# Victarry/Image-Generation-models

Measured on AMD Instinct MI355X. Metric: ddpm_cifar10_32x32_train_images_per_sec, higher is better.
Workload: dtype bf16; 1 GPU; DDPM CIFAR-10 32x32, UNet 128/1-2-4, T=1000 (BASELINE configs[1]): train step B=128/GPU + hipGraph denoise step B=64; per_gpu_batch=128, global_batch=128, parallelism=dp1, step_launch=hipGraph replay, denoise_batch=64, rccl_ranks=1, state_finite=True, matmul=bf16 MFMA, fp32 accumulate

## Files before the change

image-generation-models_amd/csrc/conv3x3_halo.hip:

```cpp
#include <stdlib.h>
#include "common.h"

#ifdef MI_HALO_TIMING
__device__ unsigned long long g_halo_ts[5 * 4096];
#define MI_TS(k) do { if (threadIdx.x == 0 && blockIdx.y == 0 && blockIdx.z == 0 && blockIdx.x < 4096) g_halo_ts[(k) * 4096 + blockIdx.x] = wall_clock64(); } while (0)
extern "C" int mi_debug_halo_ts(unsigned long long* host_out) {
    return (int)hipMemcpyFromSymbol(host_out, HIP_SYMBOL(g_halo_ts), sizeof(g_halo_ts));
}
#else
#define MI_TS(k) do {} while (0)
#endif
#ifdef MI_HALO_TAPTIME
__device__ unsigned long long g_halo_tap[4096 * 8 * 5];
extern "C" int mi_debug_halo_tap(unsigned long long* host_out) {
    return (int)hipMemcpyFromSymbol(host_out, HIP_SYMBOL(g_halo_tap), sizeof(g_halo_tap));
}
#define MI_TAP_BARRIER() do { const unsigned long long b0_ = __builtin_amdgcn_s_memtime(); __syncthreads(); \
        const unsigned long long b1_ = __builtin_amdgcn_s_memtime(); tt_work += b0_ - tt_prev; tt_bar += b1_ - b0_; tt_prev = b1_; ++tt_n; } while (0)
#else
#define MI_TAP_BARRIER() __syncthreads()
#endif
#ifndef MI_HALO_STORE_FIRST
#define MI_HALO_STORE_FIRST 1
#endif
// ... 617 lines not shown
    if (skew_env && KS == 3 && (a.W == 8 || a.W == 16)) {
        const int rows = a.TI * (a.TH + 2);
        if (a.HP * PITCH + rows * HaloSkew<CK>::EL <= MAXHP * PITCH) a.skew = HaloSkew<CK>::EL;
    }
    dim3 grid((a.N * a.H * a.W + BM - 1) / BM, (a.Nc + 127) / 128, a.ksplit);
    a.qmap = 0; a.gx = (int)grid.x; a.gy = (int)grid.y;
    static const int q_env = (int)mi_knob("MI_HALO_PQ", 1);
    if (q_env && KS == 3 && !SK && a.ksplit == 1 && !a.xmap && a.gy > 1 && a.TH == a.H) {
        const int Q = (a.gy % 2 == 0) ? 2 : 1, P = 8 / Q;
        if (Q > 1 && a.gx % P == 0) { a.qmap = Q; grid = dim3(grid.x * grid.y, 1, 1); }
    }
    if (q_env && KS == 1 && !SK && a.ksplit == 1 && a.gy > 1 && a.gx % 8 == 0) { a.qmap = 1; grid = dim3(grid.x * grid.y, 1, 1); }
    static MiPerDevice once;
    once.run([] {
        (void)hipFuncSetAttribute((const void*)conv3x3_halo_kernel<BM, CK, KS, SK, IO, WAVES, FUSE, PIPE, N64>, hipFuncAttributeMaxDynamicSharedMemorySize, 160 * 1024); });
    hipLaunchKernelGGL((conv3x3_halo_kernel<BM, CK, KS, SK, IO, WAVES, FUSE, PIPE, N64>), grid, dim3(HaloCfg<BM, WAVES>::NT), lds, st, a);
}

struct PackEntry { long long off; int taps, ci, co, tile0, frag, pad_; };

constexpr int PACK_TILE = 64;

__global__ __launch_bounds__(256) void pack_weights_kernel(const PackEntry* __restrict__ ents, int nent,
                                                           const float* __restrict__ master, uint16_t* __restrict__ wd,
                                                           uint16_t* __restrict__ wf, uint16_t* __restrict__ wdq,
                                                           uint16_t* __restrict__ wfq) {
    __shared__ float tile[PACK_TILE][PACK_TILE + 1];
    int e = 0;
    for (int hi = nent; hi - e > 1;) {
        const int mid = (e + hi) >> 1;
        if ((int)blockIdx.x >= ents[mid].tile0) e = mid; else hi = mid;
    }
    const PackEntry en = ents[e];
    int local = blockIdx.x - en.tile0;
    const int tci = (en.ci + PACK_TILE - 1) / PACK_TILE, tco = (en.co + PACK_TILE - 1) / PACK_TILE;
    int tap = local / (tci * tco);
    int rem = local - tap * (tci * tco);
    int bi = rem / tco, bj = rem - bi * tco;
    const float* src = master + en.off + (size_t)tap * en.ci * en.co;
    uint16_t* d1 = wd + en.off + (size_t)tap * en.ci * en.co;
    uint16_t* d2 = wf + en.off + (size_t)tap * en.ci * en.co;
    if (((en.ci | en.co) & 3) == 0 && (en.off & 3) == 0) {
        const int c4 = (threadIdx.x & 15) * 4, r0 = threadIdx.x >> 4;
#pragma unroll
        for (int p = 0; p < 4; ++p) {
            const int r = r0 + 16 * p, i = bi * PACK_TILE + r, j = bj * PACK_TILE + c4;
            f32x4 v = {0.f, 0.f, 0.f, 0.f};
            if (i < en.ci && j < en.co) {
                v = *reinterpret_cast<const f32x4*>(src + (size_t)i * en.co + j);
                *reinterpret_cast<u32x2*>(d1 + (size_t)i * en.co + j) = u32x2{pack_bf16(v.x, v.y), pack_bf16(v.z, v.w)};
            }
            tile[r][c4] = v.x; tile[r][c4 + 1] = v.y; tile[r][c4 + 2] = v.z; tile[r][c4 + 3] = v.w;
        }
        __syncthreads();
#pragma unroll
        for (int p = 0; p < 4; ++p) {
            const int r = r0 + 16 * p, j = bj * PACK_TILE + r, i = bi * PACK_TILE + c4;
            if (i < en.ci && j < en.co)
                *reinterpret_cast<u32x2*>(d2 + (size_t)j * en.ci + i) =
                    u32x2{pack_bf16(tile[c4][r], tile[c4 + 1][r]), pack_bf16(tile[c4 + 2][r], tile[c4 + 3][r])};
        }
        if (en.frag && wdq) {
            const int l = threadIdx.x & 63;
            const size_t tapo = (size_t)en.off + (size_t)tap * en.ci * en.co;
#pragma unroll
            for (int h = 0; h < 2; ++h) {
                const int f = (threadIdx.x >> 6) + 4 * h;
                const int r32 = (f >> 2) * 32 + (l & 31), c8 = (f & 3) * 16 + 8 * (l >> 5);
                {
                    const size_t fo = ((size_t)(bi * 2 + (f >> 2)) * (en.co / 16) + bj * 4 + (f & 3)) * 512 + l * 8;
                    *reinterpret_cast<u32x4*>(wdq + tapo + fo) =
                        u32x4{pack_bf16(tile[r32][c8], tile[r32][c8 + 1]), pack_bf16(tile[r32][c8 + 2], tile[r32][c8 + 3]),
                              pack_bf16(tile[r32][c8 + 4], tile[r32][c8 + 5]), pack_bf16(tile[r32][c8 + 6], tile[r32][c8 + 7])};
                }
                {
                    const size_t fo = ((size_t)(bj * 2 + (f >> 2)) * (en.ci / 16) + bi * 4 + (f & 3)) * 512 + l * 8;
                    *reinterpret_cast<u32x4*>(wfq + tapo + fo) =
                        u32x4{pack_bf16(tile[c8][r32], tile[c8 + 1][r32]), pack_bf16(tile[c8 + 2][r32], tile[c8 + 3][r32]),
                              pack_bf16(tile[c8 + 4][r32], tile[c8 + 5][r32]), pack_bf16(tile[c8 + 6][r32], tile[c8 + 7][r32])};
                }
            }
        }
        return;
    }
    const int tx = threadIdx.x & 63, ty = threadIdx.x >> 6;
    for (int r = ty; r < PACK_TILE; r += 4) {
        int i = bi * PACK_TILE + r, j = bj * PACK_TILE + tx;
        float v = (i < en.ci && j < en.co) ? src[(size_t)i * en.co + j] : 0.f;
        tile[r][tx] = v;
        if (i < en.ci && j < en.co) d1[(size_t)i * en.co + j] = (uint16_t)(pack_bf16(v, 0.f) & 0xffff);
    }
    __syncthreads();
    for (int r = ty; r < PACK_TILE; r += 4) {
        int j = bj * PACK_TILE + r, i = bi * PACK_TILE + tx;
        if (i < en.ci && j < en.co) d2[(size_t)j * en.ci + i] = (uint16_t)(pack_bf16(tile[tx][r], 0.f) & 0xffff);
    }
}

}

static bool halo_geom(const MiConvDesc* d, int BM, int* TH, int* TI) {
    int W = d->OW, H = d->OH;
    if (BM % W) return false;
    int rows = BM / W;
    if (rows <= H) { if (H % rows) return false; *TH = rows; *TI = 1; }
    else { if (rows % H) return false; *TH = H; *TI = rows / H; if ((long)d->N % *TI) return false; }
    int maxhp = BM == 256 ? 400 : (BM == 128 ? 288 : 160);
    return *TI * (*TH + 2) * (W + 2) <= maxhp;
}

static bool halo_ok(const MiConvDesc* d, int* bm, int* ck) {
    const bool k3 = d->KH == 3 && d->KW == 3 && d->pad == 1, k1 = d->KH == 1 && d->KW == 1 && d->pad == 0;
    if (!(k3 || k1) || d->stride != 1 || d->mode != 1) return false;
    if (d->IH != d->OH || d->IW != d->OW) return false;
    if (d->K % 32 || d->K1 % 32 || d->Nc % 4) return false;
    if (k1) {
        const long M = (long)d->N * d->OH * d->OW, nt = (d->Nc + 127) / 128;
// ... 256 lines not shown
    hipStream_t st = (hipStream_t)stream;
#define MI_FUSE_GO(IOV) \
    do { if (BM == 256 && CK == 64) launch_halo<256, 64, 3, false, IOV, 8, true>(a, st); \
         else if (BM == 256) launch_halo<256, 32, 3, false, IOV, 8, true>(a, st); \
         else if (BM == 128) launch_halo<128, 32, 3, false, IOV, 4, true>(a, st); \
         else if (CK == 64) launch_halo<64, 64, 3, false, IOV, 4, true>(a, st); \
         else launch_halo<64, 32, 3, false, IOV, 4, true>(a, st); } while (0)
    if (io == 0) MI_FUSE_GO(0); else MI_FUSE_GO(3);
#undef MI_FUSE_GO
    MI_LAUNCH_CHECK();
    return 0;
}

extern "C" int mi_conv3x3_bf16w_tile(const MiConvDesc* d, int io, int* bm, int* ck, int* sk) {
    MI_REQUIRE(d && bm && ck && sk, "null argument");
    MI_REQUIRE(halo_ok(d, bm, ck), "descriptor not supported by the halo kernel");
    int th, ti;
    *sk = (!(io & 2) && halo_splitk(d, *bm, &th, &ti)) ? 1 : 0;
    if (*sk) { *bm = 256; *ck = 64; }
    else if (halo_w8(d, *bm, &th, &ti)) { *bm = 128; *ck = 64; }
    else if (halo_wide64(d, *bm)) *ck = 64;
    return 0;
}

extern "C" int mi_conv3x3_bf16w_supported(const MiConvDesc* d) {
    int bm, ck;
    return (d && halo_ok(d, &bm, &ck)) ? 1 : 0;
}

extern "C" int mi_pack_weights_tile(void) { return PACK_TILE; }

extern "C" int mi_pack_weights_bf16(int nent, const void* entries_dev, int total_tiles, const float* master,
                                    void* wd_bf16, void* wf_bf16, void* wdq_bf16, void* wfq_bf16, void* stream) {
    MI_REQUIRE(nent > 0 && entries_dev && total_tiles > 0 && master && wd_bf16 && wf_bf16, "bad argument");
    MI_REQUIRE((wdq_bf16 == nullptr) == (wfq_bf16 == nullptr), "fragment-order copies: both or neither");
    MI_REQUIRE((((uintptr_t)wdq_bf16 | (uintptr_t)wfq_bf16) & 15) == 0, "fragment-order copies must be 16-byte aligned");
    hipLaunchKernelGGL(pack_weights_kernel, dim3(total_tiles), dim3(256), 0, (hipStream_t)stream,
                       (const PackEntry*)entries_dev, nent, master, (uint16_t*)wd_bf16, (uint16_t*)wf_bf16,
                       (uint16_t*)wdq_bf16, (uint16_t*)wfq_bf16);
    MI_LAUNCH_CHECK();
    return 0;
}
```

image-generation-models_amd/src/models/ddpm.py:

```python
from __future__ import annotations

import math
import os
from functools import partial
from typing import Dict, List, Optional, Sequence, Tuple

import numpy as np
import torch
from torch import nn

from ..ops import functional as K
from .base import BaseModel, ValidationResult

_HEADS, _DHEAD = 4, 32
_GN_GROUPS = 8


def _mode_id(name: str) -> int:
    if name not in ("fp32", "bf16"):
        raise ValueError(f"compute mode must be 'fp32' or 'bf16', got {name!r}")
    return K.MODE_BF16 if name == "bf16" else K.MODE_FP32


class _Entry:
# ... 194 lines not shown
        self.compute_mode = os.environ.get("MI_DDPM_MODE", "fp32")
        self.block_storage = os.environ.get("MI_DDPM_STORAGE", "bf16")
        self.fuse_gn_conv = os.environ.get("MI_DDPM_FUSE_GN", "auto")
        self.s2_wgrad_tr = K.debug_knob("MI_DDPM_S2_TR", "1") != "0"
        self.final_block16 = K.debug_knob("MI_DDPM_FINAL16", "1") != "0"
        self.ends16 = K.debug_knob("MI_DDPM_ENDS16", "1") != "0"
        self.dual_out = K.debug_knob("MI_DDPM_DUAL_OUT", "1") != "0"
        self.fuse_ln_qkv = K.debug_knob("MI_DDPM_FUSE_LN", "1") != "0"
        self.fuse_ln_qkv_train = K.debug_knob("MI_DDPM_FUSE_LN_TRAIN", "1") != "0"
        self.small_cin_dual = K.debug_knob("MI_DDPM_CIN_DUAL", "1") != "0"
        self.cin_dual_chores = K.debug_knob("MI_DDPM_CIN_CHORES", "1") != "0"
        self.fold_attn = K.debug_knob("MI_DDPM_FOLD_ATTN", "0") == "1"
        self.small_cout_bwd1 = K.debug_knob("MI_DDPM_COUT_BWD1", "1") != "0"
        self.fuse_final = K.debug_knob("MI_DDPM_FUSE_FINAL", "1") != "0"
        self.grad_store = K.debug_knob("MI_DDPM_GRAD_STORE", "1") != "0"
        self.accumulate_grads = False
        self.grad_ready_hook = None

        flat = torch.zeros(arch.flat_numel)
        for e in arch.entries:
            if e.init == "kaiming":
                w = torch.empty(e.shape)
                nn.init.kaiming_uniform_(w, a=math.sqrt(5))
                e.logical_view(flat).copy_(w)
            elif e.init == "ubias":
                bound = 1 / math.sqrt(e.fan_in) if e.fan_in > 0 else 0
                e.logical_view(flat).copy_(torch.empty(e.shape).uniform_(-bound, bound))
            elif e.init == "one":
                e.logical_view(flat).fill_(1.0)
        object.__setattr__(self, "_flat", flat)
        object.__setattr__(self, "_gflat", None)
        object.__setattr__(self, "_dirty", 0)
        object.__setattr__(self, "_shadow", None)
        object.__setattr__(self, "_shadow_key", None)
        object.__setattr__(self, "_shadow32", None)
        object.__setattr__(self, "_shadow32_key", None)
        object.__setattr__(self, "_zero_tab", None)
        object.__setattr__(self, "_zero_tab_retired", [])
        object.__setattr__(self, "_anchor", torch.zeros(1, requires_grad=True))
        self._plist: List[Tuple[_Entry, nn.Parameter]] = []
        for e in sorted(arch.entries, key=lambda q: q.rank):
            parts = e.key.split(".")
            node = self
            for name in parts[:-1]:
                if name not in node._modules:
                    node.add_module(name, _Node())
                node = node._modules[name]
            p = nn.Parameter(e.logical_view(flat))
            node.register_parameter(parts[-1], p)
            self._plist.append((e, p))
        self._bind(flat)

    def _bind(self, flat: torch.Tensor):
        object.__setattr__(self, "_flat", flat)
        sv = {}
        for e, p in self._plist:
            p.data = e.logical_view(flat)
            sv[e.key] = e.storage_view(flat)
        object.__setattr__(self, "_sv", sv)
        object.__setattr__(self, "_offs", {e.key: e.offset for e, _ in self._plist})
        object.__setattr__(self, "_shadow_key", None)
        object.__setattr__(self, "_shadow32_key", None)
        g = self._gflat
        if g is not None and (g.device != flat.device or g.dtype != flat.dtype):
            object.__setattr__(self, "_gflat", None)
            for _, p in self._plist:
                p.grad = None

    def _apply(self, fn, recurse=True):
        new = fn(self._flat)
        if new.dtype != torch.float32:
            raise RuntimeError("the MI355X UNet keeps fp32 master weights; use compute_mode='bf16' for bf16 math")
        if new is not self._flat:
            self._bind(new)
        return self

    @property
    def flat_params(self) -> torch.Tensor:
        return self._flat

    def mark_params_dirty(self):
        object.__setattr__(self, "_dirty", self._dirty + 1)

    def _shadows(self):
        flat = self._flat
        key = (flat.data_ptr(), flat._version, self._dirty)
        if self._shadow_key != key:
            if self._shadow is None or self._shadow[0].device != flat.device:
                ents = []
                for e in self._arch.entries:
                    if e.layout in ("conv", "convT"):
                        kh, kw, ci, co = e.storage_view(flat).shape
                        ents.append((e.offset, kh * kw, ci, co))
                table, nent, tiles = K.pack_table(ents, flat.device)
                bufs = [torch.zeros(flat.numel(), device=flat.device, dtype=torch.bfloat16) for _ in range(4)]
                object.__setattr__(self, "_shadow", (*bufs, table, nent, tiles))
            wd, wf, wdq, wfq, table, nent, tiles = self._shadow
            K.pack_weights_bf16(table, nent, tiles, flat, wd, wf, wdq, wfq)
            object.__setattr__(self, "_shadow_key", key)
        return self._shadow[:4]

    def _shadows32(self):
        flat = self._flat
        key = (flat.data_ptr(), flat._version, self._dirty)
        if getattr(self, "_shadow32_key", None) != key:
            if getattr(self, "_shadow32", None) is None or self._shadow32[0].device != flat.device:
                ents = []
                for e in self._arch.entries:
                    if e.layout in ("conv", "convT"):
                        kh, kw, ci, co = e.storage_view(flat).shape
                        ents.append((e.offset, kh * kw, ci, co))
                table, nent, tiles = K.pack_table(ents, flat.device)
                bufs = [torch.zeros(flat.numel(), device=flat.device, dtype=torch.float32) for _ in range(2)]
                object.__setattr__(self, "_shadow32", (*bufs, table, nent, tiles))
            wdq32, wfq32, table, nent, tiles = self._shadow32
            K.pack_weights_f32frag(table, nent, tiles, flat, wdq32, wfq32)
            object.__setattr__(self, "_shadow32_key", key)
        return self._shadow32[:2]

    @property
    def flat_grads(self) -> torch.Tensor:
        if self._gflat is None:
            g = torch.zeros_like(self._flat)
            object.__setattr__(self, "_gflat", g)
            gv = {}
            for e, p in self._plist:
                p.grad = e.logical_view(g)
                gv[e.key] = e.storage_view(g)
            object.__setattr__(self, "_gv", gv)
            self._build_zero_table(g.device)
        return self._gflat

    def _build_zero_table(self, device):
        skip = []
        for e in self._arch.entries:
            if e.layout in ("conv", "convT"):
                kh, kw, ci, co = e.storage_view(self._flat).shape
                if ci % 64 == 0 and co >= 32:
                    skip.append((e.offset, e.numel, e.key))
        skip.sort()
        ranges, pos = [], 0
        for off, numel, _ in skip:
            if off > pos:
                ranges.append((pos, off - pos))
            pos = off + numel
        if self._arch.flat_numel > pos:
            ranges.append((pos, self._arch.flat_numel - pos))
        if self._zero_tab is not None:
            self._zero_tab_retired.append(self._zero_tab)
        table = torch.tensor(ranges, dtype=torch.int64).reshape(-1, 2).to(device)
        object.__setattr__(self, "_zero_tab", (table, len(ranges), frozenset(k for _, _, k in skip)))

    def zero_grad(self, set_to_none: bool = False):
        if self._gflat is not None:
            self._gflat.zero_()

    def load_state_dict(self, state_dict, strict: bool = True, assign: bool = False):
        out = super().load_state_dict(state_dict, strict=strict, assign=False)
        return out

    def forward(self, x, time):
        if not x.is_cuda:
            raise RuntimeError("Unet.forward: input is not on a HIP device; this implementation has no CPU path")
        if self._flat.device != x.device:
            raise RuntimeError("Unet parameters and input are on different devices; call .to(device) first")
        if torch.is_grad_enabled() and (self.training or x.requires_grad):
            if self._anchor.device != x.device:
                object.__setattr__(self, "_anchor", torch.zeros(1, device=x.device, requires_grad=True))
            return _UnetFunction.apply(x, time, self._anchor, self)
        y, _ = self._execute(x, time, record=False)
        return y

    def _execute(self, x, time, record):
        x_in = K.nchw_to_nhwc(x.float())
        eps, tape = self.forward_nhwc(x_in, time, record)
        return K.nhwc_to_nchw(eps), tape

    @torch.no_grad()
    def time_bias_table(self, timesteps: int) -> torch.Tensor:
        A, sv, flat = self._arch, self._sv, self._flat
        if not A.with_time:
            return None
        T = int(timesteps)
        t = torch.arange(T, device=flat.device, dtype=torch.long)

        def lin(inp, w, b):
            o, i = w.shape
            y = K.small_gemm(False, True, inp, w, bias=b)
            if y is not None:
                return y
            return K.conv_igemm(inp.view(T, 1, 1, i), w, kh=1, kw=1, stride=1, pad=0, transposed=False, w_kn=False,
# ... 818 lines not shown
```

image-generation-models_amd/src/ops/functional.py:

```python
from __future__ import annotations

import ctypes as C
import functools
import os
from typing import Optional, Tuple

import torch

from .lib import ROWSUM_MAX, WGRAD_STORE, MiConvDesc, MiGnDesc, MiRowSum, MiWgradDesc, check, load_library

MODE_FP32, MODE_BF16 = 0, 1


def debug_knob(name: str, default: str) -> str:
    if os.environ.get("MI_DEBUG_KNOBS") == "1":
        return os.environ.get(name, default)
    return default
PROBE = None


CONV_AUTO = os.environ.get("MI_CONV_AUTO", "1") == "1"


USE_CONV_PW = CONV_AUTO and debug_knob("MI_CONV_PW", "1") == "1"
# ... 54 lines not shown
def _probe_open():
    if PROBE is None:
        return None
    e0 = torch.cuda.Event(enable_timing=True)
    e0.record()
    return e0


def _probe_close(e0, sym, flops, desc, nbytes=0.0):
    e1 = torch.cuda.Event(enable_timing=True)
    e1.record()
    PROBE.append((sym, float(flops), e0, e1, desc, float(nbytes)))


def _esz(t) -> int:
    return 0 if t is None else t.element_size()


def _stream() -> C.c_void_p:
    global LAUNCHES
    LAUNCHES += 1
    return C.c_void_p(_raw_stream(_cur_dev()))


LAUNCHES = 0


_cur_dev = torch._C._cuda_getDevice
_raw_stream = torch._C._cuda_getCurrentRawStream


def _p(t: Optional[torch.Tensor]) -> C.c_void_p:
    return C.c_void_p(0 if t is None else t.data_ptr())


def _need_gpu(t: torch.Tensor):
    if not t.is_cuda:
        raise RuntimeError("libmi_ddpm kernels need tensors on an MI355X (HIP) device; there is no CPU fallback")
    if t.dtype not in (torch.float32, torch.bfloat16):
        raise RuntimeError(f"expected float32 (or bf16 block-internal storage), got {t.dtype}")
    if t.device.index != _cur_dev():
        raise RuntimeError(f"tensor is on {t.device} but the current HIP device is cuda:{torch.cuda.current_device()}; "
                           "call torch.cuda.set_device(tensor.device) first (one process per GPU)")
    if t.device.index not in _SPLITK_WS:
        _splitk_workspace(t.device)


_SPLITK_WS = {}
SPLITK_MB = int(debug_knob("MI_CONV_PW_SPLITK_MB", "64"))


def _splitk_workspace(device):
    ws = None
    if SPLITK_MB > 0 and USE_CONV_PW and not torch.cuda.is_current_stream_capturing():
        ws = torch.zeros(SPLITK_MB << 20, dtype=torch.uint8, device=device)
        torch.cuda.current_stream().synchronize()
        check(load_library().mi_conv_pw_set_splitk_workspace(ws.data_ptr(), ws.numel()), "mi_conv_pw_set_splitk_workspace")
    elif torch.cuda.is_current_stream_capturing():
        return
    _SPLITK_WS[device.index] = ws


def ld_of(t: torch.Tensor) -> int:
    if t.dim() == 2:
        assert t.stride(1) == 1
        return t.stride(0)
# ... 50 lines not shown
    if e0 is not None:
        pxt, ncls = C.c_int(), C.c_int()
        load_library().mi_conv_gt_tile(C.byref(d), C.byref(pxt), C.byref(ncls))
        flops = 2.0 * N * OH * OW * Nc * K * (kh * kw if not (transposed and stride > 1) else kh * kw / (stride * stride))
        nb = N * IH * IW * K * _esz(x) + N * OH * OW * Nc * _esz(out) * (2 if accumulate else 1) + kh * kw * K * Nc * _esz(x)
        _probe_close(e0, f"conv_gt_kernel<{'true' if _b16(out) else 'false'}, {pxt.value}{', true' if mode == MODE_FP32 else ''}>", flops,
                     f"N{N} {IH}x{IW}->{OH}x{OW} K{K}->{Nc} k{kh} s{stride} T{int(transposed)} acc{int(accumulate)}", nb)
    return (out, y16) if want16 else out


def conv_igemm(x, w, *, kh, kw, stride, pad, transposed, w_kn, K, Nc, out_hw, mode, x2=None,
               bias=None, residual=None, out=None, accumulate=False, wb=None):
    _need_gpu(x)
    N, IH, IW, K1 = x.shape
    if x2 is None:
        K1 = K
    OH, OW = out_hw
    if out is None:
        assert not accumulate
        out = new_act(N, OH, OW, Nc if Nc % 4 == 0 else (Nc + 3) // 4 * 4, x)
        if out.shape[3] != Nc:
            out.zero_()
            out = out[..., :Nc]
    d = MiConvDesc(N=N, IH=IH, IW=IW, OH=OH, OW=OW, K=K, Nc=Nc, KH=kh, KW=kw, stride=stride, pad=pad,
                   transposed=int(transposed), w_kn=int(w_kn), mode=mode, K1=K1, ldx=ld_of(x),
                   ldx2=ld_of(x2) if x2 is not None else 0, ldy=ld_of(out),
                   ldr=ld_of(residual) if residual is not None else 0, accumulate=int(accumulate))
    if PROBE is not None:
        bm, bn = C.c_int(), C.c_int()
        load_library().mi_conv_igemm_tile(C.byref(d), C.byref(bm), C.byref(bn))
        flops = 2.0 * N * OH * OW * Nc * K * (kh * kw if not (transposed and stride > 1) else kh * kw / (stride * stride))
        e0 = _probe_open()
    in16 = _b16(x)
    if in16:
        if wb is None or mode != MODE_BF16 or (x2 is not None and not _b16(x2)) or not load_library().mi_conv_igemm_bf16w_io_supported(C.byref(d)):
            raise RuntimeError("bf16-stored activations: layer not supported (check igemm_bf16_in_supported first)")
        check(load_library().mi_conv_igemm_bf16w_io(C.byref(d), _p(x), _p(x2), _p(wb), _p(bias), _p(residual), _p(out), 1, _stream()),
              "mi_conv_igemm_bf16w_io")
    elif wb is not None and mode == MODE_BF16 and K % 8 == 0:
        check(load_library().mi_conv_igemm_bf16w(C.byref(d), _p(x), _p(x2), _p(wb), _p(bias), _p(residual), _p(out), _stream()),
              "mi_conv_igemm_bf16w")
    else:
        check(load_library().mi_conv_igemm(C.byref(d), _p(x), _p(x2), _p(w), _p(bias), _p(residual), _p(out), _stream()),
              "mi_conv_igemm")
    if PROBE is not None:
        fast = wb is not None and mode == MODE_BF16 and K % 8 == 0
        nb = N * IH * IW * K * _esz(x) + N * OH * OW * Nc * _esz(out) * (2 if accumulate else 1) + kh * kw * K * Nc * (2 if fast else 4)
        _probe_close(e0, f"igemm{'_fast' if fast else ''}_kernel<{mode},{bm.value},{bn.value}{',in16' if in16 else ''}>", flops,
                     f"N{N} {IH}x{IW}->{OH}x{OW} K{K}->{Nc} k{kh} s{stride} T{int(transposed)} acc{int(accumulate)}", nb)
    return out


def conv3x3_bf16w(x, wsh, *, K, Nc, flip, ksize=3, x2=None, bias=None, residual=None, out=None, accumulate=False,
                  out_dtype=torch.float32, gn_sums=None, want16=False, wq=None):
    _need_gpu(x)
    N, H, W, K1 = x.shape
    if x2 is None:
        K1 = K
    d = MiConvDesc(N=N, IH=H, IW=W, OH=H, OW=W, K=K, Nc=Nc, KH=ksize, KW=ksize, stride=1, pad=ksize // 2, transposed=int(flip),
                   w_kn=0, mode=MODE_BF16, K1=K1, ldx=ld_of(x), ldx2=ld_of(x2) if x2 is not None else 0, ldy=0,
                   ldr=ld_of(residual) if residual is not None else 0, accumulate=int(accumulate))
    lib = load_library()
    if not _query("mi_conv3x3_bf16w_supported", d):
        return None
    if out is None:
        assert not accumulate
# ... 33 lines not shown
        pt = _query("mi_conv3x3_pw_x32_tile", d)
        if pt and (N * H * W // pt) * ((Nc + 127) // 128) >= PW_MIN_TILES:
            assert gn_sums is None or (gn_sums.dtype == torch.int64 and gn_sums.numel() == N * (Nc // 16) * 2)
            e0 = _probe_open()
            check(lib.mi_conv3x3_pw_x32(C.byref(d), _p(x), _p(x2), _p(wq), _p(bias), _p(residual), _p(out), _b16(out), _p(gn_sums), _stream()),
                  "mi_conv3x3_pw_x32")
            if e0 is not None:
                nb = (N * H * W * K * 4 + N * H * W * Nc * (_esz(out) * (2 if accumulate else 1) + _esz(residual)) + 9 * K * Nc * 2)
                _probe_close(e0, f"conv_pw_kernel<{'true' if _b16(out) else 'false'}, {0 if gn_sums is None else 1}, 0, {_pw_tile_now(d, 0, True, pt)}, true>",
                             2.0 * N * H * W * Nc * K * 9, f"N{N} {H}x{W} K{K}{'(2src)' if x2 is not None else ''}->{Nc} fp32 in flip{int(flip)} acc{int(accumulate)}", nb)
            return out
    if (gn_sums is not None and ksize == 3 and _b16(x) and USE_CONV_PW and wq is not None and _pick_pw(N, H, W, K, Nc, d)
            and _query("mi_conv3x3_pw_supported", d)):
        assert gn_sums.dtype == torch.int64 and gn_sums.numel() == N * (Nc // 16) * 2
        e0 = _probe_open()
        check(lib.mi_conv3x3_pw_gnsums(C.byref(d), _p(x), _p(x2), _p(wq), _p(bias), _p(residual), _p(out), _b16(out), _p(gn_sums), _stream()),
              "mi_conv3x3_pw_gnsums")
        if e0 is not None:
            nb = (N * H * W * K * 2 + N * H * W * Nc * (_esz(out) * (2 if accumulate else 1) + _esz(residual)) + 9 * K * Nc * 2)
            _probe_close(e0, _pw_sym(d, _b16(out), 1), 2.0 * N * H * W * Nc * K * 9,
                         f"N{N} {H}x{W} K{K}->{Nc} + GroupNorm sums", nb)
        return out
    if gn_sums is None and not want16 and ksize == 3 and _b16(x):
        if USE_CONV_PW and wq is not None and _pick_pw(N, H, W, K, Nc, d):
            pick = "pw"
    if pick == "pw":
        e0 = _probe_open()
        check(lib.mi_conv3x3_pw(C.byref(d), _p(x), _p(x2), _p(wq), _p(bias), _p(residual), _p(out), _b16(out), _stream()), "mi_conv3x3_pw")
        if e0 is not None:
            nb = (N * H * W * K * 2 + N * H * W * Nc * (_esz(out) * (2 if accumulate else 1) + _esz(residual)) + 9 * K * Nc * 2)
            _probe_close(e0, _pw_sym(d, _b16(out)), 2.0 * N * H * W * Nc * K * 9,
                         f"N{N} {H}x{W} K{K}{'(2src)' if x2 is not None else ''}->{Nc} flip{int(flip)} acc{int(accumulate)}", nb)
        return out
    e0 = _probe_open()
    if want16:
        assert out.dtype == torch.float32 and gn_sums is None and not accumulate
        y16 = new_act(N, H, W, Nc, x, torch.bfloat16)
        check(lib.mi_conv3x3_bf16w_io_dual(C.byref(d), _p(x), _p(x2), _p(wsh), _p(bias), _p(residual), _p(out), _p(y16), ld_of(y16), io, _stream()),
              "mi_conv3x3_bf16w_io_dual")
    elif gn_sums is not None:
        assert ksize == 3 and gn_sums.dtype == torch.int64 and gn_sums.numel() == N * (Nc // 16) * 2
        check(lib.mi_conv3x3_bf16w_io_gnsums(C.byref(d), _p(x), _p(x2), _p(wsh), _p(bias), _p(residual), _p(out), io, _p(gn_sums), _stream()),
              "mi_conv3x3_bf16w_io_gnsums")
    elif io:
        check(lib.mi_conv3x3_bf16w_io(C.byref(d), _p(x), _p(x2), _p(wsh), _p(bias), _p(residual), _p(out), io, _stream()),
              "mi_conv3x3_bf16w_io")
    else:
        check(lib.mi_conv3x3_bf16w(C.byref(d), _p(x), _p(x2), _p(wsh), _p(bias), _p(residual), _p(out), _stream()),
              "mi_conv3x3_bf16w")
    if e0 is not None:
        bm, ck, sk = C.c_int(), C.c_int(), C.c_int()
        lib.mi_conv3x3_bf16w_tile(C.byref(d), io, C.byref(bm), C.byref(ck), C.byref(sk))
        nb = (N * H * W * K * _esz(x) + N * H * W * Nc * (_esz(out) * (2 if accumulate else 1) + _esz(residual))
              + ksize * ksize * K * Nc * 2)
        _probe_close(e0, f"conv3x3_halo_kernel<{bm.value}, {ck.value}, {ksize}, {'true' if sk.value else 'false'}, {io}, {8 if bm.value == 256 or (bm.value == 128 and ck.value == 64) else 4}>",
                     2.0 * N * H * W * Nc * K * ksize * ksize,
                     f"N{N} {H}x{W} K{K}{'(2src)' if x2 is not None else ''}->{Nc} flip{int(flip)} acc{int(accumulate)} io{io}", nb)
    return (out, y16) if want16 else out


def gn_stats_coef(x, gamma, beta, *, groups=8, eps=1e-5, temb=None):
    _need_gpu(x)
    N, H, W, Cc = x.shape
    stats = torch.empty((N, groups, 2), device=x.device, dtype=torch.float32)
    coef = torch.empty((3, N, Cc), device=x.device, dtype=torch.float32)
    d = MiGnDesc(N=N, HW=H * W, C=Cc, G=groups, eps=eps, ldx=ld_of(x), ldy=Cc, ldr=0)
# ... 95 lines not shown
                                                 _stream()), "mi_conv3x3_pw_gn_mish_sums")
        else:
            check(lib.mi_conv3x3_pw_gn_mish(C.byref(d), _p(x), _p(coef), _p(wq), _p(bias), _p(y), _b16(y), _stream()), "mi_conv3x3_pw_gn_mish")
        if e0 is not None:
            _probe_close(e0, f"conv_pw_kernel<{'true' if _b16(y) else 'false'}, {3 if coef is None else 2}, 0, {_pw_tile_now(d, 2, False, ptf)}>", 2.0 * N * H * W * Nc * K * 9,
                         f"N{N} {H}x{W} K{K}->{Nc} fused GN+Mish", N * H * W * (K * 2 + Nc * _esz(y)) + 9 * K * Nc * 2)
        return y
    if ptf and x.dtype == torch.float32:
        y = new_act(N, H, W, Nc, x, x.dtype if out_dtype is None else out_dtype)
        d.ldy = Nc
        e0 = _probe_open()
        if coef is None and (K // gn[4]) not in (16, 32, 64):
            _, coef = gn_coef_from_sums(gn[0], N, H * W, gn[1], gn[2], groups=gn[4], eps=gn[5], temb=gn[3])
        if coef is None:
            sums, gamma, beta, temb, groups, eps = gn
            check(lib.mi_conv3x3_pw_x32_gn_mish_sums(C.byref(d), _p(x), _p(sums), _p(gamma), _p(beta), _p(temb),
                                                     ld_of(temb) if temb is not None else 0, groups, eps, _p(wq), _p(bias), _p(y), _b16(y),
                                                     _stream()), "mi_conv3x3_pw_x32_gn_mish_sums")
        else:
            check(lib.mi_conv3x3_pw_x32_gn_mish(C.byref(d), _p(x), _p(coef), _p(wq), _p(bias), _p(y), _b16(y), _stream()),
                  "mi_conv3x3_pw_x32_gn_mish")
        if e0 is not None:
            _probe_close(e0, f"conv_pw_kernel<{'true' if _b16(y) else 'false'}, {3 if coef is None else 2}, 0, {_pw_tile_now(d, 2, True, ptf)}, true>",
                         2.0 * N * H * W * Nc * K * 9, f"N{N} {H}x{W} K{K}->{Nc} fused GN+Mish, fp32 in",
                         N * H * W * (K * 4 + Nc * _esz(y)) + 9 * K * Nc * 2)
        return y
    if not lib.mi_conv3x3_gn_mish_supported(C.byref(d)):
        return None
    out_dtype = x.dtype if out_dtype is None else out_dtype
    if out_dtype != x.dtype:
        raise RuntimeError("the fused kernel writes y in x's storage type (fp32 -> fp32 or bf16 -> bf16)")
    y = new_act(N, H, W, Nc, x, out_dtype)
    io = 3 if x.dtype == torch.bfloat16 else 0
    e0 = _probe_open()
    if gn is not None:
        sums, gamma, beta, temb, groups, eps = gn
        check(lib.mi_conv3x3_gn_mish_sums(C.byref(d), _p(x), _p(sums), _p(gamma), _p(beta), _p(temb), ld_of(temb) if temb is not None else 0,
                                          groups, eps, _p(wsh), _p(bias), _p(y), io, _stream()), "mi_conv3x3_gn_mish_sums")
    else:
        check(lib.mi_conv3x3_gn_mish(C.byref(d), _p(x), _p(coef), _p(wsh), _p(bias), _p(y), io, _stream()), "mi_conv3x3_gn_mish")
    if e0 is not None:
        bm, ck = C.c_int(), C.c_int()
        lib.mi_conv3x3_gn_mish_tile(C.byref(d), C.byref(bm), C.byref(ck))
        _probe_close(e0, f"conv3x3_halo_kernel<{bm.value}, {ck.value}, 3, false, {io}, {8 if bm.value == 256 else 4}, true>",
                     2.0 * N * H * W * Nc * K * 9, f"N{N} {H}x{W} K{K}->{Nc} fused GN+Mish",
                     N * H * W * (K * _esz(x) + Nc * _esz(y)) + 9 * K * Nc * 2)
    return y


def pack_weights_tile():
    return int(load_library().mi_pack_weights_tile())


PACK_ENTRY = [("off", "<i8"), ("taps", "<i4"), ("ci", "<i4"), ("co", "<i4"), ("tile0", "<i4"), ("frag", "<i4"), ("pad", "<i4")]


def pack_table(entries, device):
    import numpy as np
    rec = np.zeros(len(entries), dtype=np.dtype(PACK_ENTRY))
    tile, T = 0, pack_weights_tile()
    for i, (off, taps, ci, co) in enumerate(entries):
        rec[i] = (off, taps, ci, co, tile, int(taps in (1, 9, 16) and ci % 64 == 0 and co % 64 == 0), 0)
        tile += taps * ((ci + T - 1) // T) * ((co + T - 1) // T)
    return torch.from_numpy(rec.view(np.uint8).copy()).to(device), len(entries), tile


def pack_weights_bf16(table_dev, nent, total_tiles, master, wd, wf, wdq=None, wfq=None):
    e0 = _probe_open()
    check(load_library().mi_pack_weights_bf16(nent, _p(table_dev), total_tiles, _p(master), _p(wd), _p(wf), _p(wdq), _p(wfq), _stream()),
          "mi_pack_weights_bf16")
    if e0 is not None:
        _probe_close(e0, "pack_weights_kernel", 0.0, f"{master.numel()} params", master.numel() * (8.0 if wdq is None else 12.0))


def pack_weights_f32frag(table_dev, nent, total_tiles, master, wdq32, wfq32):
    e0 = _probe_open()
    check(load_library().mi_pack_weights_f32frag(nent, _p(table_dev), total_tiles, _p(master), _p(wdq32), _p(wfq32), _stream()),
          "mi_pack_weights_f32frag")
    if e0 is not None:
        _probe_close(e0, "pack_f32frag_kernel", 0.0, f"{master.numel()} params", master.numel() * 12.0)


def conv3x3_f32(x, wq32, *, K, Nc, flip, x2=None, bias=None, residual=None, out=None, accumulate=False):
    _need_gpu(x)
    if x.dtype != torch.float32 or (x2 is not None and x2.dtype != torch.float32) or not USE_CONV_PW:
        return None
    N, H, W, K1 = x.shape
    if x2 is None:
        K1 = K
    d = MiConvDesc(N=N, IH=H, IW=W, OH=H, OW=W, K=K, Nc=Nc, KH=3, KW=3, stride=1, pad=1, transposed=int(flip),
                   w_kn=0, mode=MODE_FP32, K1=K1, ldx=ld_of(x), ldx2=ld_of(x2) if x2 is not None else 0, ldy=Nc,
                   ldr=ld_of(residual) if residual is not None else 0, accumulate=int(accumulate))
    pt = _query("mi_conv3x3_pw_f32_tile", d)
    if not pt:
        return None
    if out is None:
        assert not accumulate
        out = new_act(N, H, W, Nc, x, torch.float32)
    d.ldy = ld_of(out)
    if d.ldy % 8:
        return None
    e0 = _probe_open()
    check(load_library().mi_conv3x3_pw_f32(C.byref(d), _p(x), _p(x2), _p(wq32), _p(bias), _p(residual), _p(out), _stream()), "mi_conv3x3_pw_f32")
    if e0 is not None:
        nb = (N * H * W * K * 4 + N * H * W * Nc * (4 * (2 if accumulate else 1) + _esz(residual)) + 9 * K * Nc * 4)
# ... 674 lines not shown
    M, D = src_rows.shape
    check(load_library().mi_vq_scatter_rows(M, D, table.shape[0], _p(src_rows), src_rows.stride(0), _p(idx), _p(table), _stream()),
          "mi_vq_scatter_rows")


def linattn_fwd(qkv, heads=4):
    _need_gpu(qkv)
    N, H, W, C3 = qkv.shape
    assert C3 == 3 * heads * 32 and qkv.is_contiguous()
    out = new_act(N, H, W, heads * 32, qkv, qkv.dtype)
    ctx = torch.empty((N, heads, 32, 32), device=qkv.device, dtype=torch.float32)
    kstat = torch.empty((N, heads, 32, 2), device=qkv.device, dtype=torch.float32)
    e0 = _probe_open()
    lib = load_library()
    need = _linattn_ws(N, H * W, heads)
    ws = _workspace(qkv.device, need) if need else None
    check(lib.mi_linattn_fwd_ws(N, H * W, heads, _p(qkv), _p(out), _p(ctx), _p(kstat), _b16(qkv), _p(ws), ws.numel() * 4 if need else 0,
                                _stream()), "mi_linattn_fwd")
    if e0 is not None:
        _probe_close(e0, f"linattn_fwd_kernel<io{_b16(qkv)}>", 4.0 * N * heads * 32 * 32 * H * W, f"N{N} n{H * W}",
                     N * H * W * heads * 32 * 4 * _esz(qkv))
    return out, ctx, kstat


def linattn_to_out_folded(qkv, w_out16, Cc, bias, residual, heads=4, want16=False):
    _need_gpu(qkv)
    N, H, W, C3 = qkv.shape
    hid = heads * 32
    if (qkv.dtype != torch.bfloat16 or C3 != 3 * hid or not qkv.is_contiguous() or hid % 128 or Cc % 64 or (H * W) % 64 or (N * H * W) % 128
            or _linattn_ws(N, H * W, heads)):
        return None
    lib = load_library()
    weff = torch.empty((N, Cc * hid), device=qkv.device, dtype=torch.bfloat16)
    e0 = _probe_open()
    check(lib.mi_linattn_fold_fwd(N, H * W, heads, _p(qkv), _p(w_out16), Cc, _p(weff), _stream()), "mi_linattn_fold_fwd")
    if e0 is not None:
        _probe_close(e0, "linattn_fwd_kernel<io1, fold>", 2.0 * N * heads * 32 * 32 * (H * W + Cc), f"N{N} n{H * W} C{Cc}",
                     N * H * W * 2 * hid * 2 + N * Cc * hid * 2)
    y = new_act(N, H, W, Cc, qkv, torch.float32)
    y16 = new_act(N, H, W, Cc, qkv, torch.bfloat16) if want16 else None
    d = MiConvDesc(N=N, IH=H, IW=W, OH=H, OW=W, K=hid, Nc=Cc, KH=1, KW=1, stride=1, pad=0, transposed=0, w_kn=0, mode=MODE_BF16, K1=hid,
                   ldx=C3, ldx2=0, ldy=ld_of(y), ldr=ld_of(residual) if residual is not None else 0, accumulate=0)
    e0 = _probe_open()
    check(lib.mi_conv1x1_pw_batched(C.byref(d), _p(qkv), _p(weff), Cc * hid, _p(bias), _p(residual), _p(y), 0, _p(y16),
                                    ld_of(y16) if y16 is not None else 0, _stream()), "mi_conv1x1_pw_batched")
    if e0 is not None:
        px = 64 if ((N * H * W // 128) * ((Cc + 127) // 128) < 256 or (H * W) % 128) else 128
        _probe_close(e0, f"conv1x1_pw_kernel<false, {'true' if want16 else 'false'}, {px}>", 2.0 * N * H * W * Cc * hid,
                     f"N{N} {H}x{W} K{hid}->{Cc} per-sample weights", N * H * W * (hid * 2 + Cc * (4 + _esz(residual) + (2 if want16 else 0))) + N * Cc * hid * 2)
    return (y, y16) if want16 else y


def linattn_bwd(qkv, ctx, kstat, dout, heads=4):
    N, H, W, C3 = qkv.shape
    assert dout.is_contiguous() and dout.dtype == qkv.dtype
    dqkv = torch.empty_like(qkv)
    e0 = _probe_open()
    lib = load_library()
    need = _linattn_ws(N, H * W, heads)
    ws = _workspace(qkv.device, need) if need else None
    check(lib.mi_linattn_bwd_ws(N, H * W, heads, _p(qkv), _p(ctx), _p(kstat), _p(dout), _p(dqkv), _b16(qkv), _p(ws),
                                ws.numel() * 4 if need else 0, _stream()), "mi_linattn_bwd")
    if e0 is not None:
        _probe_close(e0, f"linattn_bwd_kernel<io{_b16(qkv)}>", 12.0 * N * heads * 32 * 32 * H * W, f"N{N} n{H * W}",
                     N * H * W * heads * 32 * 7 * _esz(qkv))
    return dqkv
# ... 760 lines not shown
```

image-generation-models_amd/src/runtime/graphed.py:

```python
from __future__ import annotations

import torch


def _new_graph():
    try:
        return torch.cuda.CUDAGraph(keep_graph=True)
    except TypeError:
        return torch.cuda.CUDAGraph()


def node_types(g):
    try:
        import collections
        import ctypes
        hip = ctypes.CDLL("libamdhip64.so")
        names = {0: "kernel", 1: "memcpy", 2: "memset", 3: "host", 4: "graph", 5: "empty", 6: "waitEvent", 7: "eventRecord"}
        raw = g.raw_cuda_graph()
        n = ctypes.c_size_t(0)
        if hip.hipGraphGetNodes(ctypes.c_void_p(raw), None, ctypes.byref(n)) != 0:
            return None
        arr = (ctypes.c_void_p * n.value)()
        if hip.hipGraphGetNodes(ctypes.c_void_p(raw), arr, ctypes.byref(n)) != 0:
            return None
        c = collections.Counter()
        for i in range(n.value):
            t = ctypes.c_int(-1)
            hip.hipGraphNodeGetType(ctypes.c_void_p(arr[i]), ctypes.byref(t))
            c[names.get(t.value, str(t.value))] += 1
        return dict(c)
    except Exception:
        return None


class GraphedTrainStep:
    def __init__(self, model, optimizer, example_batch, warmup: int = 3):
        self.model, self.opt = model, optimizer
        imgs = example_batch[0]
        self.x = imgs.clone()
        self.rest = tuple(r.clone() if torch.is_tensor(r) else r for r in example_batch[1:])
        s = torch.cuda.Stream()
        s.wait_stream(torch.cuda.current_stream())
        with torch.cuda.stream(s):
            for i in range(warmup):
                loss = model.training_step((self.x,) + self.rest, i)
                loss.backward()
                optimizer.step()
        torch.cuda.current_stream().wait_stream(s)
        self.graph = _new_graph()
        with torch.cuda.graph(self.graph):
            self.loss = model.training_step((self.x,) + self.rest, 0)
            self.loss.backward()
            optimizer.step()
        self.warmup_steps = warmup

    def __call__(self, batch):
        self.x.copy_(batch[0], non_blocking=True)
        for dst, src in zip(self.rest, batch[1:]):
            if torch.is_tensor(dst) and torch.is_tensor(src) and dst.shape == src.shape:
                dst.copy_(src, non_blocking=True)
        self.graph.replay()
        for n in getattr(self.opt, "nets", ()):
            n.mark_params_dirty()
        return self.loss


class SegmentedGraphedTrainStep:

    def __init__(self, model, optimizer, reducer, example_batch):
        self.model, self.opt, self.red = model, optimizer, reducer
        self.x = example_batch[0].clone()
        self.rest = tuple(example_batch[1:])
        self.segments = []
        self.pool = torch.cuda.graph_pool_handle()
        self._cur = None
        optimizer.device_state = True
        dev = self.x.device
        self.stream = torch.cuda.Stream(dev)
        self.stream.wait_stream(torch.cuda.current_stream(dev))
        with torch.cuda.stream(self.stream):
            reducer.begin()
            reducer.capture_sink = self._cut
            try:
                self._final = False
                self._begin()
                self.loss = model.training_step_and_backward((self.x,) + self.rest, 0)
                self._final = True
                reducer.finish()
                if self._cur is not None:
                    self._end(None)
            except BaseException:
                if self._cur is not None:
                    try:
                        self._cur.capture_end()
                    except Exception:
                        pass
                    self._cur = None
                raise
            finally:
                reducer.capture_sink = None
            self.adam = torch.cuda.CUDAGraph()
            self.adam.capture_begin(pool=self.pool)
            optimizer.step()
            self.adam.capture_end()
        torch.cuda.current_stream(dev).wait_stream(self.stream)
        self.logged = {}

    def _begin(self):
        self._cur = _new_graph()
        self._cur.capture_begin(pool=self.pool)

    @staticmethod
    def _node_count(g):
        nt = node_types(g)
        return None if nt is None else sum(nt.values())

    def _end(self, rng):
        self._cur.capture_end()
        if rng is None and self._node_count(self._cur) == 0:
            self._cur = None
            return
        self.segments.append((self._cur, rng))
        self._cur = None

    def _cut(self, lo, hi):
        self._end((lo, hi))
        if not self._final:
            self._begin()

    def __call__(self, batch):
        self.x.copy_(batch[0], non_blocking=True)
        self.red.begin()
        for g, rng in self.segments:
            g.replay()
            if rng is not None:
                self.red.launched.append(rng)
                self.red.all_reduce_async(*rng)
        self.red.wait_all()
        self.adam.replay()
        for n in getattr(self.opt, "nets", ()):
            n.mark_params_dirty()
        return self.loss
```

image-generation-models_amd/src/runtime/sampler.py:

```python
from __future__ import annotations

import torch

from ..ops import functional as K


class GraphSampler:
    def __init__(self, gd, shape):
        self.gd, self.shape = gd, tuple(shape)
        dev = gd.betas.device
        self.x = torch.zeros(shape, device=dev)
        self.xh_full = torch.zeros((shape[0], shape[2], shape[3], (shape[1] + 3) // 4 * 4), device=dev)
        self.xh = self.xh_full[..., :shape[1]]
        self.z = torch.zeros(shape, device=dev)
        self.t = torch.zeros((shape[0],), device=dev, dtype=torch.long)
        self.one = torch.ones((shape[0],), device=dev, dtype=torch.long)
        self.graph = None
        self.tb_table = None

    def _iteration(self):
        gd = self.gd
        if K.debug_knob("MI_SAMPLER_INPLACE", "1") != "1":
            eps, _ = gd.denoise_fn.forward_nhwc(K.nchw_to_nhwc(self.x), self.t, record=False, time_bias_table=self.tb_table)
            xp, _ = K.p_sample_update(self.x, eps, self.z, self.t, gd._tables(), clip=True, want_nhwc=False)
            self.x.copy_(xp)
            self.t.sub_(self.one)
            return
        eps, _ = gd.denoise_fn.forward_nhwc(self.xh, self.t, record=False, time_bias_table=self.tb_table)
        K.p_sample_update(self.x, eps, self.z, self.t, gd._tables(), clip=True, out=self.x, out_nhwc=self.xh_full)
        self.t.sub_(self.one)

    def set_image(self, x):
        self.x.copy_(x)
        self.xh.copy_(K.nchw_to_nhwc(self.x))

    def refresh(self):
        net = self.gd.denoise_fn
        if getattr(net, "compute_mode", "fp32") == "bf16":
            net._shadows()
        tab = net.time_bias_table(self.gd.num_timesteps)
        if self.tb_table is None:
            self.tb_table = tab
        else:
            self.tb_table.copy_(tab)

    def _capture(self):
        self.refresh()
        s = torch.cuda.Stream()
        s.wait_stream(torch.cuda.current_stream())
        with torch.cuda.stream(s):
            self.t.fill_(1)
            self.set_image(torch.zeros_like(self.x))
            self._iteration()
        torch.cuda.current_stream().wait_stream(s)
        self.graph = torch.cuda.CUDAGraph()
        with torch.cuda.graph(self.graph):
            self._iteration()

    @torch.no_grad()
    def run(self, record=None):
        gd = self.gd
        if self.graph is None:
            self._capture()
        else:
            self.refresh()
        self.set_image(gd._randn(self.shape, self.x.device))
        self.t.fill_(gd.num_timesteps - 1)
        for _ in range(gd.num_timesteps):
            if gd.noise_source is None:
                self.z.normal_()
            else:
                self.z.copy_(gd._randn(self.shape, self.x.device))
# ... 5 lines not shown
```

Baseline: 27320 images/s.

## Pack plain bf16 weight shadows lazily, only when a consumer requests them

Splits weight-shadow packing into fragment-order and plain copies with separate freshness keys. Plain copies are handed out as lazy PlainShadow handles and are packed only when a layer actually needs them, or when the previous weight generation asked for them. This is meant to cut the per-step bf16 pack write traffic when only fragment-order weights are used. The graph guard refreshes whichever shadows were live at capture time before each replay, which adds host-side bookkeeping and risks stale plain shadows if the tracking is wrong.

```diff
diff --git a/image-generation-models_amd/csrc/conv3x3_halo.hip b/image-generation-models_amd/csrc/conv3x3_halo.hip
--- a/image-generation-models_amd/csrc/conv3x3_halo.hip
+++ b/image-generation-models_amd/csrc/conv3x3_halo.hip
@@ -673,14 +673,15 @@
         if ((int)blockIdx.x >= ents[mid].tile0) e = mid; else hi = mid;
     }
     const PackEntry en = ents[e];
+    if (!wd && !(en.frag && wdq)) return;
     int local = blockIdx.x - en.tile0;
     const int tci = (en.ci + PACK_TILE - 1) / PACK_TILE, tco = (en.co + PACK_TILE - 1) / PACK_TILE;
     int tap = local / (tci * tco);
     int rem = local - tap * (tci * tco);
     int bi = rem / tco, bj = rem - bi * tco;
     const float* src = master + en.off + (size_t)tap * en.ci * en.co;
-    uint16_t* d1 = wd + en.off + (size_t)tap * en.ci * en.co;
-    uint16_t* d2 = wf + en.off + (size_t)tap * en.ci * en.co;
+    uint16_t* d1 = wd ? wd + en.off + (size_t)tap * en.ci * en.co : nullptr;
+    uint16_t* d2 = wd ? wf + en.off + (size_t)tap * en.ci * en.co : nullptr;
     if (((en.ci | en.co) & 3) == 0 && (en.off & 3) == 0) {
         const int c4 = (threadIdx.x & 15) * 4, r0 = threadIdx.x >> 4;
 #pragma unroll
@@ -689,7 +690,7 @@
             f32x4 v = {0.f, 0.f, 0.f, 0.f};
             if (i < en.ci && j < en.co) {
                 v = *reinterpret_cast<const f32x4*>(src + (size_t)i * en.co + j);
-                *reinterpret_cast<u32x2*>(d1 + (size_t)i * en.co + j) = u32x2{pack_bf16(v.x, v.y), pack_bf16(v.z, v.w)};
+                if (d1) *reinterpret_cast<u32x2*>(d1 + (size_t)i * en.co + j) = u32x2{pack_bf16(v.x, v.y), pack_bf16(v.z, v.w)};
             }
             tile[r][c4] = v.x; tile[r][c4 + 1] = v.y; tile[r][c4 + 2] = v.z; tile[r][c4 + 3] = v.w;
         }
@@ -697,7 +698,7 @@
 #pragma unroll
         for (int p = 0; p < 4; ++p) {
             const int r = r0 + 16 * p, j = bj * PACK_TILE + r, i = bi * PACK_TILE + c4;
-            if (i < en.ci && j < en.co)
+            if (d2 && i < en.ci && j < en.co)
                 *reinterpret_cast<u32x2*>(d2 + (size_t)j * en.ci + i) =
                     u32x2{pack_bf16(tile[c4][r], tile[c4 + 1][r]), pack_bf16(tile[c4 + 2][r], tile[c4 + 3][r])};
         }
@@ -724,6 +725,7 @@
         }
         return;
     }
+    if (!d1) return;
     const int tx = threadIdx.x & 63, ty = threadIdx.x >> 6;
     for (int r = ty; r < PACK_TILE; r += 4) {
         int i = bi * PACK_TILE + r, j = bj * PACK_TILE + tx;
@@ -1046,8 +1048,10 @@
 
 extern "C" int mi_pack_weights_bf16(int nent, const void* entries_dev, int total_tiles, const float* master,
                                     void* wd_bf16, void* wf_bf16, void* wdq_bf16, void* wfq_bf16, void* stream) {
-    MI_REQUIRE(nent > 0 && entries_dev && total_tiles > 0 && master && wd_bf16 && wf_bf16, "bad argument");
+    MI_REQUIRE(nent > 0 && entries_dev && total_tiles > 0 && master, "bad argument");
+    MI_REQUIRE((wd_bf16 == nullptr) == (wf_bf16 == nullptr), "plain copies: both or neither");
     MI_REQUIRE((wdq_bf16 == nullptr) == (wfq_bf16 == nullptr), "fragment-order copies: both or neither");
+    MI_REQUIRE(wd_bf16 || wdq_bf16, "nothing to write: neither plain nor fragment-order copies given");
     MI_REQUIRE((((uintptr_t)wdq_bf16 | (uintptr_t)wfq_bf16) & 15) == 0, "fragment-order copies must be 16-byte aligned");
     hipLaunchKernelGGL(pack_weights_kernel, dim3(total_tiles), dim3(256), 0, (hipStream_t)stream,
                        (const PackEntry*)entries_dev, nent, master, (uint16_t*)wd_bf16, (uint16_t*)wf_bf16,
diff --git a/image-generation-models_amd/src/models/ddpm.py b/image-generation-models_amd/src/models/ddpm.py
--- a/image-generation-models_amd/src/models/ddpm.py
+++ b/image-generation-models_amd/src/models/ddpm.py
@@ -250,7 +250,10 @@
         object.__setattr__(self, "_gflat", None)
         object.__setattr__(self, "_dirty", 0)
         object.__setattr__(self, "_shadow", None)
-        object.__setattr__(self, "_shadow_key", None)
+        object.__setattr__(self, "_frag_key", None)
+        object.__setattr__(self, "_plain_key", None)
+        object.__setattr__(self, "_wgen", 0)
+        object.__setattr__(self, "_plain_ask", -1)
         object.__setattr__(self, "_shadow32", None)
         object.__setattr__(self, "_shadow32_key", None)
         object.__setattr__(self, "_zero_tab", None)
@@ -277,7 +280,8 @@
             sv[e.key] = e.storage_view(flat)
         object.__setattr__(self, "_sv", sv)
         object.__setattr__(self, "_offs", {e.key: e.offset for e, _ in self._plist})
-        object.__setattr__(self, "_shadow_key", None)
+        object.__setattr__(self, "_frag_key", None)
+        object.__setattr__(self, "_plain_key", None)
         object.__setattr__(self, "_shadow32_key", None)
         g = self._gflat
         if g is not None and (g.device != flat.device or g.dtype != flat.dtype):
@@ -300,23 +304,57 @@
     def mark_params_dirty(self):
         object.__setattr__(self, "_dirty", self._dirty + 1)
 
+    def _weights_key(self):
+        flat = self._flat
+        return (flat.data_ptr(), flat._version, self._dirty)
+
+    def _pack_state(self):
+        flat = self._flat
+        if self._shadow is None or self._shadow[0].device != flat.device:
+            ents = []
+            for e in self._arch.entries:
+                if e.layout in ("conv", "convT"):
+                    kh, kw, ci, co = e.storage_view(flat).shape
+                    ents.append((e.offset, kh * kw, ci, co))
+            table, nent, tiles = K.pack_table(ents, flat.device)
+            bufs = [torch.zeros(flat.numel(), device=flat.device, dtype=torch.bfloat16) for _ in range(4)]
+            object.__setattr__(self, "_shadow", (*bufs, table, nent, tiles))
+            object.__setattr__(self, "_frag_key", None)
+            object.__setattr__(self, "_plain_key", None)
+        return self._shadow
+
+    def _new_weights(self):
+        want = self._plain_ask == self._wgen
+        object.__setattr__(self, "_wgen", self._wgen + 1)
+        return want
+
+    def refresh_shadows(self, plain=False):
+        wd, wf, wdq, wfq, table, nent, tiles = self._pack_state()
+        key = self._weights_key()
+        frag_stale, plain_stale = self._frag_key != key, self._plain_key != key
+        if frag_stale and self._new_weights():
+            plain = True
+        plain = plain and plain_stale
+        if frag_stale or plain:
+            K.pack_weights_bf16(table, nent, tiles, self._flat, wd if plain else None, wf if plain else None,
+                                wdq if frag_stale else None, wfq if frag_stale else None)
+            if frag_stale:
+                object.__setattr__(self, "_frag_key", key)
+            if plain:
+                object.__setattr__(self, "_plain_key", key)
+
+    def shadows_fresh(self):
+        key = self._weights_key()
+        return (self._shadow is not None and self._frag_key == key, self._shadow is not None and self._plain_key == key)
+
+    def plain_shadows(self):
+        self.refresh_shadows(plain=True)
+        object.__setattr__(self, "_plain_ask", self._wgen)
+        return self._shadow[0], self._shadow[1]
+
     def _shadows(self):
-        flat = self._flat
-        key = (flat.data_ptr(), flat._version, self._dirty)
-        if self._shadow_key != key:
-            if self._shadow is None or self._shadow[0].device != flat.device:
-                ents = []
-                for e in self._arch.entries:
-                    if e.layout in ("conv", "convT"):
-                        kh, kw, ci, co = e.storage_view(flat).shape
-                        ents.append((e.offset, kh * kw, ci, co))
-                table, nent, tiles = K.pack_table(ents, flat.device)
-                bufs = [torch.zeros(flat.numel(), device=flat.device, dtype=torch.bfloat16) for _ in range(4)]
-                object.__setattr__(self, "_shadow", (*bufs, table, nent, tiles))
-            wd, wf, wdq, wfq, table, nent, tiles = self._shadow
-            K.pack_weights_bf16(table, nent, tiles, flat, wd, wf, wdq, wfq)
-            object.__setattr__(self, "_shadow_key", key)
-        return self._shadow[:4]
+        self.refresh_shadows()
+        return K.PlainShadow(self, 0), K.PlainShadow(self, 1), self._shadow[2], self._shadow[3]
 
     def _shadows32(self):
         flat = self._flat
@@ -375,6 +413,7 @@
 
     def load_state_dict(self, state_dict, strict: bool = True, assign: bool = False):
         out = super().load_state_dict(state_dict, strict=strict, assign=False)
+        self.mark_params_dirty()
         return out
 
     def forward(self, x, time):
diff --git a/image-generation-models_amd/src/ops/functional.py b/image-generation-models_amd/src/ops/functional.py
--- a/image-generation-models_amd/src/ops/functional.py
+++ b/image-generation-models_amd/src/ops/functional.py
@@ -110,6 +110,25 @@
 
 def _p(t: Optional[torch.Tensor]) -> C.c_void_p:
     return C.c_void_p(0 if t is None else t.data_ptr())
+
+
+class PlainShadow:
+    __slots__ = ("owner", "which", "off")
+
+    def __init__(self, owner, which, off=0):
+        self.owner, self.which, self.off = owner, which, off
+
+    def __getitem__(self, sl):
+        if not isinstance(sl, slice) or sl.stop is not None or sl.step is not None or (sl.start or 0) < 0:
+            raise IndexError("a plain weight shadow is sliced as w[offset:]")
+        return PlainShadow(self.owner, self.which, self.off + (sl.start or 0))
+
+    def tensor(self):
+        return self.owner.plain_shadows()[self.which][self.off:]
+
+
+def _plain(w):
+    return w.tensor() if isinstance(w, PlainShadow) else w
 
 
 def _need_gpu(t: torch.Tensor):
@@ -226,6 +245,8 @@
         flops = 2.0 * N * OH * OW * Nc * K * (kh * kw if not (transposed and stride > 1) else kh * kw / (stride * stride))
         e0 = _probe_open()
     in16 = _b16(x)
+    if wb is not None and mode == MODE_BF16 and (in16 or K % 8 == 0):
+        wb = _plain(wb)
     if in16:
         if wb is None or mode != MODE_BF16 or (x2 is not None and not _b16(x2)) or not load_library().mi_conv_igemm_bf16w_io_supported(C.byref(d)):
             raise RuntimeError("bf16-stored activations: layer not supported (check igemm_bf16_in_supported first)")
@@ -325,6 +346,7 @@
             _probe_close(e0, _pw_sym(d, _b16(out)), 2.0 * N * H * W * Nc * K * 9,
                          f"N{N} {H}x{W} K{K}{'(2src)' if x2 is not None else ''}->{Nc} flip{int(flip)} acc{int(accumulate)}", nb)
         return out
+    wsh = _plain(wsh)
     e0 = _probe_open()
     if want16:
         assert out.dtype == torch.float32 and gn_sums is None and not accumulate
@@ -486,6 +508,7 @@
         raise RuntimeError("the fused kernel writes y in x's storage type (fp32 -> fp32 or bf16 -> bf16)")
     y = new_act(N, H, W, Nc, x, out_dtype)
     io = 3 if x.dtype == torch.bfloat16 else 0
+    wsh = _plain(wsh)
     e0 = _probe_open()
     if gn is not None:
         sums, gamma, beta, temb, groups, eps = gn
@@ -524,7 +547,9 @@
     check(load_library().mi_pack_weights_bf16(nent, _p(table_dev), total_tiles, _p(master), _p(wd), _p(wf), _p(wdq), _p(wfq), _stream()),
           "mi_pack_weights_bf16")
     if e0 is not None:
-        _probe_close(e0, "pack_weights_kernel", 0.0, f"{master.numel()} params", master.numel() * (8.0 if wdq is None else 12.0))
+        kinds = ("plain" if wd is not None else "") + ("+" if wd is not None and wdq is not None else "") + ("frag" if wdq is not None else "")
+        _probe_close(e0, "pack_weights_kernel", 0.0, f"{master.numel()} params {kinds}",
+                     master.numel() * (4.0 + (4.0 if wd is not None else 0.0) + (4.0 if wdq is not None else 0.0)))
 
 
 def pack_weights_f32frag(table_dev, nent, total_tiles, master, wdq32, wfq32):
@@ -1265,6 +1290,7 @@
         return None
     lib = load_library()
     weff = torch.empty((N, Cc * hid), device=qkv.device, dtype=torch.bfloat16)
+    w_out16 = _plain(w_out16)
     e0 = _probe_open()
     check(lib.mi_linattn_fold_fwd(N, H * W, heads, _p(qkv), _p(w_out16), Cc, _p(weff), _stream()), "mi_linattn_fold_fwd")
     if e0 is not None:
diff --git a/image-generation-models_amd/src/runtime/graphed.py b/image-generation-models_amd/src/runtime/graphed.py
--- a/image-generation-models_amd/src/runtime/graphed.py
+++ b/image-generation-models_amd/src/runtime/graphed.py
@@ -33,6 +33,26 @@
         return None
 
 
+class _ShadowGuard:
+
+    def __init__(self, opt):
+        self.opt = opt
+        self.entry = [(n, n.shadows_fresh()) for n in getattr(opt, "nets", ()) if hasattr(n, "shadows_fresh")]
+
+    def before_replay(self):
+        for n, (frag, plain) in self.entry:
+            if frag or plain:
+                n.refresh_shadows(plain=plain)
+
+    def after_capture(self):
+        for n, _ in self.entry:
+            n.mark_params_dirty()
+
+    def after_replay(self):
+        for n in getattr(self.opt, "nets", ()):
+            n.mark_params_dirty()
+
+
 class GraphedTrainStep:
     def __init__(self, model, optimizer, example_batch, warmup: int = 3):
         self.model, self.opt = model, optimizer
@@ -47,11 +67,13 @@
                 loss.backward()
                 optimizer.step()
         torch.cuda.current_stream().wait_stream(s)
+        self.guard = _ShadowGuard(optimizer)
         self.graph = _new_graph()
         with torch.cuda.graph(self.graph):
             self.loss = model.training_step((self.x,) + self.rest, 0)
             self.loss.backward()
             optimizer.step()
+        self.guard.after_capture()
         self.warmup_steps = warmup
 
     def __call__(self, batch):
@@ -59,9 +81,9 @@
         for dst, src in zip(self.rest, batch[1:]):
             if torch.is_tensor(dst) and torch.is_tensor(src) and dst.shape == src.shape:
                 dst.copy_(src, non_blocking=True)
+        self.guard.before_replay()
         self.graph.replay()
-        for n in getattr(self.opt, "nets", ()):
-            n.mark_params_dirty()
+        self.guard.after_replay()
         return self.loss
 
 
@@ -79,6 +101,7 @@
         self.stream = torch.cuda.Stream(dev)
         self.stream.wait_stream(torch.cuda.current_stream(dev))
         with torch.cuda.stream(self.stream):
+            self.guard = _ShadowGuard(optimizer)
             reducer.begin()
             reducer.capture_sink = self._cut
             try:
@@ -103,6 +126,7 @@
             self.adam.capture_begin(pool=self.pool)
             optimizer.step()
             self.adam.capture_end()
+            self.guard.after_capture()
         torch.cuda.current_stream(dev).wait_stream(self.stream)
         self.logged = {}
 
@@ -130,6 +154,7 @@
 
     def __call__(self, batch):
         self.x.copy_(batch[0], non_blocking=True)
+        self.guard.before_replay()
         self.red.begin()
         for g, rng in self.segments:
             g.replay()
@@ -138,6 +163,5 @@
                 self.red.all_reduce_async(*rng)
         self.red.wait_all()
         self.adam.replay()
-        for n in getattr(self.opt, "nets", ()):
-            n.mark_params_dirty()
+        self.guard.after_replay()
         return self.loss
diff --git a/image-generation-models_amd/src/runtime/sampler.py b/image-generation-models_amd/src/runtime/sampler.py
--- a/image-generation-models_amd/src/runtime/sampler.py
+++ b/image-generation-models_amd/src/runtime/sampler.py
@@ -37,7 +37,7 @@
     def refresh(self):
         net = self.gd.denoise_fn
         if getattr(net, "compute_mode", "fp32") == "bf16":
-            net._shadows()
+            net.refresh_shadows(plain=True)
         tab = net.time_bias_table(self.gd.num_timesteps)
         if self.tb_table is None:
             self.tb_table = tab
```

Result: no change. 27530 images/s (median of 6 runs) (+0.8%).
